# hbdat/cvpr22_cross_modal_pseudo_labeling

Measured on AMD Instinct MI355X. Metric: images/sec student-teacher train step (COCO 800x1333), higher is better.
Workload: dtype f32 (bf16x3 split MFMA, fp32 accum); 1 GPU; student_teacher_mask_rcnn_uncertainty.yaml R-50-C4, 2 img/GPU 3x800x1333, fwd+bwd+allreduce+SGD; global_batch=2, parallelism=dp1, losses_finite=True, pipelined=True

## Files before the change

cvpr22_cross_modal_pseudo_labeling_amd/csrc/ovis_common.h:

```cpp
#pragma once
#include <hip/hip_runtime.h>
#include <stdint.h>

#include "ovis_hip.h"

#define OVIS_HIP_TRY(expr)                         \
  do {                                             \
    hipError_t _e = (expr);                        \
    if (_e != hipSuccess) return (int)_e;          \
  } while (0)

#define OVIS_LAUNCH_CHECK()                        \
  do {                                             \
    hipError_t _e = hipGetLastError();             \
    if (_e != hipSuccess) return (int)_e;          \
  } while (0)

static inline int ovis_ceil_div(long a, long b) { return (int)((a + b - 1) / b); }

#define OVIS_NUM_CU 256
#define OVIS_WAVE 64
```

cvpr22_cross_modal_pseudo_labeling_amd/csrc/split_gemm.hip:

```cpp
#include <stdlib.h>

#include "ovis_common.h"
constexpr int kGroupWidth = 4;

namespace {
typedef short bf16x8 __attribute__((ext_vector_type(8)));
typedef float f32x4 __attribute__((ext_vector_type(4)));
typedef __bf16 b2 __attribute__((ext_vector_type(2)));
typedef float f2 __attribute__((ext_vector_type(2)));

__device__ char g_zero_line[128];

enum { PLAIN = 0, SHIFTED = 1, HALO = 2, DEFORM = 3 };
constexpr int kHalo = 8;

struct SplitGemmArgs {
  const char* A; long a_rs;
  const char* A2; long a2_rs;
  const char* B; long b_rs;
  float* C; long ldc;
  char* Cp; long cp_rs;
  const float* bias; const float* res; long ldr;
  const char* resp; long resp_rs;
  const char* gate; long gate_rs;
  float* pool; int pool_rows; float pool_scale;
  float* slab;
  long M; int N; int ch; int ch2; int T; int H; int W; int KH; int KW; int flip; int relu; int gw;
  int kslices; int steps_per_slice;
  const float* dimg; const float* doff; const float* dmask;
  int Ho; int Wo; int sh; int sw; int ph; int pw; int dlh; int dlw; int dg;
};

__device__ __forceinline__ void glds16(const char* gsrc, char* lds_wave_base) {
  __builtin_amdgcn_global_load_lds((const __attribute__((address_space(1))) void*)gsrc,
                                   (__attribute__((address_space(3))) void*)lds_wave_base, 16, 0, 0);
}

__device__ __forceinline__ unsigned pack_bf16(float a, float b) {
  f2 v = {a, b};
  return __builtin_bit_cast(unsigned, __builtin_convertvector(v, b2));
}

struct EpilogueOperands {
  uint2 a, b;
};

struct EpilogueSource {
  const char* base;
  long row_bytes;
  int second;
};

__device__ __forceinline__ EpilogueSource epilogue_source(const SplitGemmArgs& p) {
// ... 427 lines not shown
            if constexpr (POOL) {
              const int rr = f * 16 + r;
              const f32x4 z = {0.f, 0.f, 0.f, 0.f};
              ps0 += rr < pool_b1 ? fin : z;
              ps1 += (rr >= pool_b1 && rr < pool_b2) ? fin : z;
              ps2 += rr >= pool_b2 ? fin : z;
            }
          }
        }
      }
    }
  }
  if constexpr (POOL) {
    f32x4* ps[3] = {&ps0, &ps1, &ps2};
#pragma unroll
    for (int sgm = 0; sgm < 3; ++sgm) {
      f32x4 v = *ps[sgm];
#pragma unroll
      for (int e = 0; e < 4; ++e) {
        v[e] += __shfl_xor(v[e], 16, 64);
        v[e] += __shfl_xor(v[e], 32, 64);
      }
      const long first = (m0 + wm * 64) + (sgm == 0 ? 0 : (sgm == 1 ? pool_b1 : pool_b2));
      if (er == 0 && col_ok && first < p.M && (sgm == 0 || (sgm == 1 ? pool_b1 : pool_b2) < 64)) {
        float* d = p.pool + (pool_map0 + sgm) * p.N + n;
#pragma unroll
        for (int e = 0; e < 4; ++e) atomicAdd(d + e, v[e] * p.pool_scale);
      }
    }
  }
}

__global__ __launch_bounds__(256) void split_gemm_finish_kernel(SplitGemmArgs p) {
  const int n4 = p.N >> 2;
  const long total = p.M * n4;
  const long slab = p.M * p.N;
  for (long i = (long)blockIdx.x * 256 + threadIdx.x; i < total; i += (long)gridDim.x * 256) {
    const long m = i / n4;
    const int n = (int)(i - m * n4) * 4;
    const float* s = p.slab + m * p.N + n;
    f32x4 v = *(const f32x4*)s;
    for (int k = 1; k < p.kslices; ++k) v += *(const f32x4*)(s + k * slab);
    epilogue_store4(p, m, n, v);
  }
}

typedef short bf16x4 __attribute__((ext_vector_type(4)));

struct SplitGemmTnArgs {
  const char* G; long g_rs;
  const char* X; long x_rs;
  float* C;
  long M; int N; int ch; int T; int H; int W; int KH; int KW; int slices; int steps_per_slice;
  int g_major;
};

#define OVIS_TR_READ(dst, addr, off) \
  asm volatile("ds_read_b64_tr_b16 %0, %1 offset:%2" : "=v"(dst) : "v"(addr), "n"(off) : "memory")
#define OVIS_LGKM_WAIT8(N, a, b, c, d, e, f, g, h)                                                                \
  asm volatile("s_waitcnt lgkmcnt(%8)"                                                                             \
               : "+v"(a), "+v"(b), "+v"(c), "+v"(d), "+v"(e), "+v"(f), "+v"(g), "+v"(h)                            \
               : "n"(N)                                                                                            \
               : "memory")

template <bool CONV, bool SMALL = false>
__global__ __launch_bounds__(256, 2) void split_gemm_tn_kernel(SplitGemmTnArgs p, int tiles_i, int tiles_j,
                                                              int nblocks) {
  constexpr int TILE_BYTES = 32 * 512, STAGE = 2 * TILE_BYTES;
  extern __shared__ __attribute__((aligned(16))) char smem[];
  const int lane = threadIdx.x & 63, wave = threadIdx.x >> 6;
  int id;
  {
    constexpr int kChunk = 2 * OVIS_NUM_CU;
    const int b = blockIdx.x, base = b / kChunk * kChunk;
    const int nb = min(nblocks - base, kChunk), bl = b - base;
    const int q = nb >> 3, r = nb & 7, xcd = bl & 7, loc = bl >> 3;
    id = base + (xcd < r ? xcd * (q + 1) : r * (q + 1) + (xcd - r) * q) + loc;
  }
  const int per_slice = tiles_i * tiles_j;
  const int slice = id / per_slice;
  const int rem = id - slice * per_slice;
  const int tile_j = p.g_major ? rem % tiles_j : rem / tiles_i;
  const int tile_i = p.g_major ? rem / tiles_j : rem - tile_j * tiles_i;
  const int i0 = tile_i * 128, j0 = tile_j * 128;
  const int tap = CONV ? j0 / p.ch : 0, c0 = CONV ? j0 - tap * p.ch : j0;
  int off_rows = 0, tdy = 0, tdx = 0;
  if (CONV) {
    tdy = tap / p.KW - p.KH / 2;
    tdx = tap % p.KW - p.KW / 2;
    off_rows = tdy * p.W + tdx;
  }
  const long step0 = (long)slice * p.steps_per_slice;
  const long steps_total = (p.M + 31) >> 5;
  long step1 = step0 + p.steps_per_slice;
  if (step1 > steps_total) step1 = steps_total;
  const int nk = step1 > step0 ? (int)(step1 - step0) : 0;

  const int prow = lane >> 5, pseg = (lane & 31) >> 1, phalf = lane & 1;
  int rows[4];
  long g_off[4], x_off[4];
  int x_y[4], x_x[4];
  int m_row[4];
  const int HW = CONV ? p.H * p.W : 1;
  unsigned long long tap_mask = 0;
  if (CONV && SMALL) {
    const int qy = lane / p.W, qx = lane - qy * p.W;
    tap_mask = __ballot(lane < HW && (unsigned)(qy + tdy) < (unsigned)p.H && (unsigned)(qx + tdx) < (unsigned)p.W);
  }
#pragma unroll
  for (int i = 0; i < 4; ++i) {
    const int piece = wave * 4 + i;
    const int row = piece * 2 + prow;
    rows[i] = row;
    const int fr = (((row >> 3) & 1) << 2) | (row & 3);
    const int seg = pseg ^ fr;
    const int m = (int)(step0 << 5) + row;
    m_row[i] = m;
    g_off[i] = (long)m * p.g_rs + (long)i0 * 4 + seg * 32 + phalf * 16;
    x_off[i] = ((long)m + off_rows) * p.x_rs + (long)c0 * 4 + seg * 32 + phalf * 16;
    x_x[i] = CONV ? (SMALL ? m % HW : m % p.W) : 0;
    x_y[i] = (CONV && !SMALL) ? (m / p.W) % p.H : 0;
  }
  const int step_q = (CONV && SMALL) ? 32 % HW : 0;
  const int step_dx = CONV ? 32 % p.W : 0, step_dy = CONV ? 32 / p.W : 0;
  const bool y_single = step_dy + 1 <= p.H;
  const char* zero_src = g_zero_line + (lane & 7) * 16;
  const int Mi = (int)p.M;

  auto issue = [&](int stage) {
    char* base = smem + stage * STAGE;
    bool x_ok[4];
#pragma unroll
    for (int i = 0; i < 4; ++i) {
      x_ok[i] = m_row[i] < Mi;
      if (CONV && SMALL) {
        x_ok[i] = x_ok[i] && ((tap_mask >> x_x[i]) & 1ull) != 0ull;
        int q = x_x[i] + step_q;
        if (q >= HW) q -= HW;
        x_x[i] = q;
      } else if (CONV) {
        x_ok[i] = x_ok[i] && (unsigned)(x_y[i] + tdy) < (unsigned)p.H && (unsigned)(x_x[i] + tdx) < (unsigned)p.W;
        int x = x_x[i] + step_dx, y = x_y[i] + step_dy;
        if (x >= p.W) { x -= p.W; ++y; }
        if (y_single) { if (y >= p.H) y -= p.H; } else { y %= p.H; }
        x_x[i] = x;
        x_y[i] = y;
      }
    }
#pragma unroll
    for (int i = 0; i < 4; ++i) {
      const char* src = p.G + g_off[i];
      if (m_row[i] >= Mi) src = zero_src;
      glds16(src, base + (wave * 4 + i) * 1024);
      g_off[i] += 32 * p.g_rs;
    }
#pragma unroll
    for (int i = 0; i < 4; ++i) {
      const char* src = p.X + x_off[i];
      if (!x_ok[i]) src = zero_src;
      glds16(src, base + TILE_BYTES + (wave * 4 + i) * 1024);
      x_off[i] += 32 * p.x_rs;
      m_row[i] += 32;
    }
  };

  const int wi = wave >> 1, wj = wave & 1;
  const int gq = lane >> 4, pp = lane & 15;
  const int rrow = 8 * gq + (pp >> 2);
  const int rfr = ((gq & 1) << 2) | (pp >> 2);
  int g_rd[4], x_rd[4];
#pragma unroll
  for (int f = 0; f < 4; ++f) {
    const int seg_g = (2 * wi + (f >> 1)) * 4 + (f & 1);
    g_rd[f] = rrow * 512 + ((seg_g ^ rfr) << 5) + (pp & 3) * 8;
    const int seg_x = (2 * wj + (f >> 1)) * 4 + (f & 1);
    x_rd[f] = TILE_BYTES + rrow * 512 + ((seg_x ^ rfr) << 5) + (pp & 3) * 8;
  }

  f32x4 acc[4][4];
#pragma unroll
  for (int f = 0; f < 4; ++f)
#pragma unroll
    for (int g = 0; g < 4; ++g) acc[f][g] = f32x4{0.f, 0.f, 0.f, 0.f};

  if (nk > 0) issue(0);
  for (int kb = 0; kb < nk; ++kb) {
    __syncthreads();
    if (kb + 1 < nk) issue((kb + 1) & 1);
    const int so = (kb & 1) * STAGE;
    bf16x4 xa[4][2], xb[4][2], ga[4][2], gb[4][2];
#pragma unroll
    for (int f = 0; f < 4; ++f) {
      const int ax = so + x_rd[f], ag = so + g_rd[f];
      OVIS_TR_READ(xa[f][0], ax, 0);
      OVIS_TR_READ(xb[f][0], ax, 2048);
      OVIS_TR_READ(ga[f][0], ag, 0);
      OVIS_TR_READ(gb[f][0], ag, 2048);
    }
#pragma unroll
    for (int f = 0; f < 4; ++f) {
      const int ax = so + (x_rd[f] ^ 64), ag = so + (g_rd[f] ^ 64);
      OVIS_TR_READ(xa[f][1], ax, 0);
      OVIS_TR_READ(xb[f][1], ax, 2048);
      OVIS_TR_READ(ga[f][1], ag, 0);
      OVIS_TR_READ(gb[f][1], ag, 2048);
    }
    OVIS_LGKM_WAIT8(15, xa[0][0], xb[0][0], ga[0][0], gb[0][0], xa[1][0], xb[1][0], ga[1][0], gb[1][0]);
    OVIS_LGKM_WAIT8(15, xa[2][0], xb[2][0], ga[2][0], gb[2][0], xa[3][0], xb[3][0], ga[3][0], gb[3][0]);
    bf16x8 gh[4], gl[4], xh[4], xl[4];
#pragma unroll
    for (int f = 0; f < 4; ++f) {
      xh[f] = __builtin_shufflevector(xa[f][0], xb[f][0], 0, 1, 2, 3, 4, 5, 6, 7);
      gh[f] = __builtin_shufflevector(ga[f][0], gb[f][0], 0, 1, 2, 3, 4, 5, 6, 7);
    }
#pragma unroll
    for (int f = 0; f < 4; ++f)
#pragma unroll
      for (int g = 0; g < 4; ++g)
        acc[f][g] = __builtin_amdgcn_mfma_f32_16x16x32_bf16(xh[g], gh[f], acc[f][g], 0, 0, 0);
    OVIS_LGKM_WAIT8(0, xa[0][1], xb[0][1], ga[0][1], gb[0][1], xa[1][1], xb[1][1], ga[1][1], gb[1][1]);
    OVIS_LGKM_WAIT8(0, xa[2][1], xb[2][1], ga[2][1], gb[2][1], xa[3][1], xb[3][1], ga[3][1], gb[3][1]);
#pragma unroll
    for (int f = 0; f < 4; ++f) {
      xl[f] = __builtin_shufflevector(xa[f][1], xb[f][1], 0, 1, 2, 3, 4, 5, 6, 7);
      gl[f] = __builtin_shufflevector(ga[f][1], gb[f][1], 0, 1, 2, 3, 4, 5, 6, 7);
    }
#pragma unroll
    for (int f = 0; f < 4; ++f)
#pragma unroll
      for (int g = 0; g < 4; ++g)
        acc[f][g] = __builtin_amdgcn_mfma_f32_16x16x32_bf16(xh[g], gl[f], acc[f][g], 0, 0, 0);
#pragma unroll
    for (int f = 0; f < 4; ++f)
#pragma unroll
      for (int g = 0; g < 4; ++g)
        acc[f][g] = __builtin_amdgcn_mfma_f32_16x16x32_bf16(xl[g], gh[f], acc[f][g], 0, 0, 0);
  }

  const long ld = (long)p.T * p.ch;
  float* out = p.C + (long)slice * p.N * ld;
#pragma unroll
// ... 350 lines not shown

extern "C" int ovis_split_gemm_tn_slices(long m, int n, int channels, int taps) {
  if (m <= 0 || n <= 0 || channels <= 0 || taps <= 0) return 1;
  const long tiles = (long)(n / 128) * ((long)taps * channels / 128);
  const long steps = (m + 31) / 32;
  if (tiles <= 0) return 1;
  const long slots = 2L * OVIS_NUM_CU;
  if (steps >= 128 && steps <= 1100 && tiles <= 64) {
    long s = slots / tiles;
    if (s > steps / 16) s = steps / 16;
    if (s > 256) s = 256;
    return (int)(s < 1 ? 1 : s);
  }
  long s_max = (4 * slots + tiles - 1) / tiles;
  if (s_max > steps / 8) s_max = steps / 8;
  if (s_max > 256) s_max = 256;
  if (s_max < 1) s_max = 1;
  long best = 1;
  double best_score = -1.0;
  for (long s = 1; s <= s_max; ++s) {
    const long blocks = s * tiles, rounds = (blocks + slots - 1) / slots;
    double score = (double)blocks / (double)(rounds * slots);
    if (rounds == 1) score *= 0.97 * (double)blocks / (double)slots;
    if (rounds > 2) score -= 0.01 * (double)(rounds - 2);
    if (score > best_score + 1e-9) { best_score = score; best = s; }
  }
  return (int)best;
}

extern "C" int ovis_split_gemm_pair_tn(const void* g_pair, long g_row_bytes, const void* x_pair, long x_row_bytes,
                                       float* c_slabs, int slices, long m, int n, int channels, int taps_h,
                                       int taps_w, int height, int width, void* stream) {
  if (m < 0 || n <= 0 || channels <= 0 || taps_h <= 0 || taps_w <= 0 || !(taps_h & 1) || !(taps_w & 1) || slices <= 0)
    return OVIS_EINVAL;
  if (!g_pair || !x_pair || !c_slabs || m > 0x7fffff00L) return OVIS_EINVAL;
  const int T = taps_h * taps_w;
  if (T > 1 && (height <= 0 || width <= 0)) return OVIS_EINVAL;
  if (n % 128 != 0 || channels % 128 != 0 ||
      g_row_bytes % 16 != 0 || x_row_bytes % 16 != 0 || ((uintptr_t)g_pair & 15) || ((uintptr_t)x_pair & 15) ||
      ((uintptr_t)c_slabs & 15))
    return OVIS_ERANGE;
  SplitGemmTnArgs p;
  p.G = (const char*)g_pair; p.g_rs = g_row_bytes; p.X = (const char*)x_pair; p.x_rs = x_row_bytes;
  p.C = c_slabs; p.M = m; p.N = n; p.ch = channels; p.T = T; p.H = height; p.W = width; p.KH = taps_h; p.KW = taps_w;
  p.slices = slices;
  const long steps = (m + 31) / 32;
  p.steps_per_slice = (int)((steps + slices - 1) / slices);
  const int tiles_i = n / 128, tiles_j = (int)((long)T * channels / 128);
  p.g_major = tiles_i >= channels / 128 ? 1 : 0;
  const long nblocks = (long)tiles_i * tiles_j * slices;
  if (nblocks > 0x7fffffffL) return OVIS_ERANGE;
  hipStream_t s = (hipStream_t)stream;
  const int lds = 2 * 2 * 32 * 512;
  if (T > 1 && (long)height * width <= 64) {
    static bool attr_set_s = false;
    if (!attr_set_s) {
      OVIS_HIP_TRY(hipFuncSetAttribute((const void*)split_gemm_tn_kernel<true, true>, hipFuncAttributeMaxDynamicSharedMemorySize, lds));
      attr_set_s = true;
    }
    hipLaunchKernelGGL((split_gemm_tn_kernel<true, true>), dim3((unsigned)nblocks), dim3(256), lds, s, p, tiles_i, tiles_j, (int)nblocks);
  } else if (T > 1) {
    static bool attr_set_c = false;
    if (!attr_set_c) {
      OVIS_HIP_TRY(hipFuncSetAttribute((const void*)split_gemm_tn_kernel<true>, hipFuncAttributeMaxDynamicSharedMemorySize, lds));
      attr_set_c = true;
    }
    hipLaunchKernelGGL(split_gemm_tn_kernel<true>, dim3((unsigned)nblocks), dim3(256), lds, s, p, tiles_i, tiles_j, (int)nblocks);
  } else {
    static bool attr_set = false;
    if (!attr_set) {
      OVIS_HIP_TRY(hipFuncSetAttribute((const void*)split_gemm_tn_kernel<false>, hipFuncAttributeMaxDynamicSharedMemorySize, lds));
      attr_set = true;
    }
    hipLaunchKernelGGL(split_gemm_tn_kernel<false>, dim3((unsigned)nblocks), dim3(256), lds, s, p, tiles_i, tiles_j, (int)nblocks);
  }
  OVIS_LAUNCH_CHECK();
  return OVIS_OK;
}

namespace {
struct SplitGemmPlan {
  int mode, narrow, stages, kslices, steps_per_slice, tiles_m, tiles_n;
};

SplitGemmPlan split_gemm_plan(long m, int n, int channels, int channels2, int taps_h, int taps_w, int width, int config) {
  SplitGemmPlan q;
  const int T = taps_h * taps_w;
  q.narrow = n <= 64;
  const int bn = q.narrow ? 64 : 128;
  q.tiles_m = (int)((m + 127) / 128);
  q.tiles_n = (n + bn - 1) / bn;
  const long nb = (long)q.tiles_m * q.tiles_n;
  q.mode = PLAIN;
  if (T > 1) q.mode = (!q.narrow && !(config & 4) && (taps_h / 2) * width + taps_w / 2 <= kHalo && T <= 16) ? HALO : SHIFTED;
  const int cpb = channels / 32;
  const int units = q.mode == HALO ? cpb : T * cpb + channels2 / 32;
  q.kslices = 1;
  q.steps_per_slice = units;
  bool sliced_two_stage = false;
  if (!(config & 8) && !q.narrow && nb <= OVIS_NUM_CU / 2) {
    const int min_units = q.mode == HALO ? 1 : 8;
    long s = units / min_units;
    const long want = (2L * OVIS_NUM_CU + nb - 1) / nb;
    if (s > want) s = want;
    if (s > 64) s = 64;
    if (s >= 2) {
      q.steps_per_slice = (int)((units + s - 1) / s);
// ... 275 lines not shown
```

cvpr22_cross_modal_pseudo_labeling_amd/csrc/roi_align.hip:

```cpp
#include <stdlib.h>

#include "ovis_common.h"
#include "roi_geom.h"

namespace {
using namespace ovis_roi;

constexpr int kThreads = 256;
constexpr int kCPB = 32;
constexpr int kMaxBatch = 16;
constexpr int kFwdLdsFloats = 4352;


template <int NCS>
__device__ __forceinline__ void fwd_pool(const float* src, int cs, int rs, int oy, int ox,
                                         const RoiGeom& g, int H, int W, int PH, int PW,
                                         float* __restrict__ out_c0) {
  const int PHPW = PH * PW;
  for (int bin = threadIdx.x; bin < PHPW; bin += kThreads) {
    const int ph = bin / PW;
    const int pw = bin - ph * PW;
    float acc[NCS];
#pragma unroll
    for (int c = 0; c < NCS; ++c) acc[c] = 0.f;
// ... 253 lines not shown
    t_xrow = (t_bin - ph * PW) * g.gw;
  }
  while (c < c_end) {
    const int left = c_end - c;
    const float* plane = img + (long)c * HW;
    float* o = out_r + (long)c * PHPW;
    const int n = min(left, cs_max);
    if (tables && n >= 16) {
      fwd_batch_lds4_tab<16>(win, plane, HW, W, g, wh, ww, PHPW, ytab, xtab, t_bin, t_yrow, t_xrow, o);
      c += 16;
    } else if (tables && n >= 8) {
      fwd_batch_lds4_tab<8>(win, plane, HW, W, g, wh, ww, PHPW, ytab, xtab, t_bin, t_yrow, t_xrow, o);
      c += 8;
    } else if (tables && n >= 4) {
      fwd_batch_lds4_tab<4>(win, plane, HW, W, g, wh, ww, PHPW, ytab, xtab, t_bin, t_yrow, t_xrow, o);
      c += 4;
    } else if (n >= 16) {
      fwd_batch_lds4<16>(win, plane, HW, W, H, g, wh, ww, PH, PW, o);
      c += 16;
    } else if (n >= 8) {
      fwd_batch_lds4<8>(win, plane, HW, W, H, g, wh, ww, PH, PW, o);
      c += 8;
    } else if (n >= 4) {
      fwd_batch_lds4<4>(win, plane, HW, W, H, g, wh, ww, PH, PW, o);
      c += 4;
    } else if (n >= 2) {
      fwd_batch_lds<2>(win, plane, HW, W, H, g, wh, ww, PH, PW, o);
      c += 2;
    } else if (n == 1) {
      fwd_batch_lds<1>(win, plane, HW, W, H, g, wh, ww, PH, PW, o);
      c += 1;
    } else {
      fwd_pool<1>(plane, HW, W, 0, 0, g, H, W, PH, PW, o);
      c += 1;
    }
  }
}

typedef __bf16 pool_b2 __attribute__((ext_vector_type(2)));
typedef float pool_f2 __attribute__((ext_vector_type(2)));
__device__ __forceinline__ unsigned pool_pack_bf16(float a, float b) {
  pool_f2 v = {a, b};
  return __builtin_bit_cast(unsigned, __builtin_convertvector(v, pool_b2));
}
__device__ __forceinline__ void pool_store4_pair(char* pair_r, long obin, int c, int C, f4 o) {
  const unsigned h01 = pool_pack_bf16(o.x, o.y), h23 = pool_pack_bf16(o.z, o.w);
  const unsigned l01 = pool_pack_bf16(o.x - __uint_as_float(h01 << 16), o.y - __uint_as_float(h01 & 0xffff0000u));
  const unsigned l23 = pool_pack_bf16(o.z - __uint_as_float(h23 << 16), o.w - __uint_as_float(h23 & 0xffff0000u));
  char* d = pair_r + obin * 4L * C + (long)(c >> 5) * 128 + (c & 31) * 2;
  *(uint2*)d = make_uint2(h01, h23);
  *(uint2*)(d + 64) = make_uint2(l01, l23);
}

template <int NCS, bool FAST>
__device__ __forceinline__ void fwd_pool4_strided(const f4* win4, int rs, const RoiGeom& g, int H, int W, int bs,
                                                  int OH, int OW, float* __restrict__ out_rc, int C,
                                                  char* pair_r = nullptr, int c_abs = 0) {
  constexpr int NG = NCS / 4;
  constexpr int SG = kFwdLdsFloats / NCS;
  const int items = OH * OW * NG;
  for (int item = threadIdx.x; item < items; item += kThreads) {
    const int k = item % NG, obin = item / NG;
    const int oh = obin / OW;
    const int ph = oh * bs, pw = (obin - oh * OW) * bs;
    const f4* base = win4 + k * SG;
    f4 acc = (f4)(0.f);
    for (int iy = 0; iy < g.gh; ++iy) {
      const float y = sample_coord_t<FAST>(g.start_h, ph, g.bin_h, iy, g.gh, g.inv_gh);
      int yl, yh;
      float ly, hy;
      if (!axis_sample(y, H, yl, yh, ly, hy)) continue;
      const int ryl = (yl - g.wy0) * rs, ryh = (yh - g.wy0) * rs;
      for (int ix = 0; ix < g.gw; ++ix) {
        const float x = sample_coord_t<FAST>(g.start_w, pw, g.bin_w, ix, g.gw, g.inv_gw);
        int xl, xh;
        float lx, hx;
        if (!axis_sample(x, W, xl, xh, lx, hx)) continue;
        const float w1 = hy * hx, w2 = hy * lx, w3 = ly * hx, w4 = ly * lx;
        acc += w1 * base[ryl + (xl - g.wx0)] + w2 * base[ryl + (xh - g.wx0)] + w3 * base[ryh + (xl - g.wx0)] +
               w4 * base[ryh + (xh - g.wx0)];
      }
    }
    const f4 o = FAST ? acc * g.inv_count : acc / g.count;
    if (pair_r) pool_store4_pair(pair_r, obin, c_abs + 4 * k, C, o);
    else *(f4*)(out_rc + (long)obin * C + 4 * k) = o;
  }
}

template <bool FAST>
__device__ __forceinline__ void pool_nhwc_strided(const f4* __restrict__ img4, const RoiGeom& g, int H, int W, int C4,
                                                  int bs, int OH, int OW, float* __restrict__ out_r, char* pair_r,
                                                  int k0 = 0, int KT = -1) {
  if (KT < 0) KT = C4;
  const int items = OH * OW * KT;
  const int C = C4 * 4;
  if (g.gh == 2 && g.gw == 2) {
    for (int item = threadIdx.x; item < items; item += kThreads) {
      const int k = k0 + item % KT, obin = item / KT;
      const int oh = obin / OW;
      const int ph = oh * bs, pw = (obin - oh * OW) * bs;
      const f4* base = img4 + k;
      int yl[2], yh[2], xl[2], xh[2];
      float ly[2], hy[2], lx[2], hx[2];
      bool oky[2], okx[2];
#pragma unroll
      for (int i = 0; i < 2; ++i) {
        oky[i] = axis_sample(sample_coord_t<FAST>(g.start_h, ph, g.bin_h, i, 2, g.inv_gh), H, yl[i], yh[i], ly[i], hy[i]);
        okx[i] = axis_sample(sample_coord_t<FAST>(g.start_w, pw, g.bin_w, i, 2, g.inv_gw), W, xl[i], xh[i], lx[i], hx[i]);
      }
      const bool same_rows = oky[0] && oky[1] && yl[0] == yl[1] && yh[0] == yh[1];
      const bool same_cols = okx[0] && okx[1] && xl[0] == xl[1] && xh[0] == xh[1];
      f4 t[2][2][4];
      auto load4 = [&](int iy, int ix) {
        const long ryl = (long)yl[iy] * W * C4, ryh = (long)yh[iy] * W * C4;
        const long cl = (long)xl[ix] * C4, ch = (long)xh[ix] * C4;
        t[iy][ix][0] = base[ryl + cl];
        t[iy][ix][1] = base[ryl + ch];
        t[iy][ix][2] = base[ryh + cl];
        t[iy][ix][3] = base[ryh + ch];
      };
      auto copy4 = [&](int iy, int ix, int sy, int sx) {
#pragma unroll
        for (int q = 0; q < 4; ++q) t[iy][ix][q] = t[sy][sx][q];
      };
      if (oky[0] && okx[0]) load4(0, 0);
      if (oky[0] && okx[1]) { if (same_cols) copy4(0, 1, 0, 0); else load4(0, 1); }
      if (oky[1] && okx[0]) { if (same_rows) copy4(1, 0, 0, 0); else load4(1, 0); }
      if (oky[1] && okx[1]) {
        if (same_rows) copy4(1, 1, 0, 1);
        else if (same_cols) copy4(1, 1, 1, 0);
        else load4(1, 1);
      }
      f4 acc = (f4)(0.f);
#pragma unroll
      for (int iy = 0; iy < 2; ++iy) {
        if (!oky[iy]) continue;
#pragma unroll
        for (int ix = 0; ix < 2; ++ix) {
          if (!okx[ix]) continue;
          const float w1 = hy[iy] * hx[ix], w2 = hy[iy] * lx[ix], w3 = ly[iy] * hx[ix], w4 = ly[iy] * lx[ix];
          acc += w1 * t[iy][ix][0] + w2 * t[iy][ix][1] + w3 * t[iy][ix][2] + w4 * t[iy][ix][3];
// ... 5 lines not shown
    }
    return;
  }
  for (int item = threadIdx.x; item < items; item += kThreads) {
    const int k = k0 + item % KT, obin = item / KT;
    const int oh = obin / OW;
    const int ph = oh * bs, pw = (obin - oh * OW) * bs;
    const f4* base = img4 + k;
    f4 acc = (f4)(0.f);
    for (int iy = 0; iy < g.gh; ++iy) {
      const float y = sample_coord_t<FAST>(g.start_h, ph, g.bin_h, iy, g.gh, g.inv_gh);
      int yl, yh;
      float ly, hy;
      if (!axis_sample(y, H, yl, yh, ly, hy)) continue;
      const long ryl = (long)yl * W * C4, ryh = (long)yh * W * C4;
      for (int ix = 0; ix < g.gw; ++ix) {
        const float x = sample_coord_t<FAST>(g.start_w, pw, g.bin_w, ix, g.gw, g.inv_gw);
        int xl, xh;
        float lx, hx;
        if (!axis_sample(x, W, xl, xh, lx, hx)) continue;
        const float w1 = hy * hx, w2 = hy * lx, w3 = ly * hx, w4 = ly * lx;
        const long cl = (long)xl * C4, ch = (long)xh * C4;
        acc += w1 * base[ryl + cl] + w2 * base[ryl + ch] + w3 * base[ryh + cl] + w4 * base[ryh + ch];
      }
    }
    const f4 o = FAST ? acc * g.inv_count : acc / g.count;
    if (pair_r) pool_store4_pair(pair_r, obin, 4 * k, C, o);
    else *(f4*)(out_r + (long)obin * C + 4 * k) = o;
  }
}

__global__ __launch_bounds__(kThreads) void roi_align_fwd_nhwc_in_strided_kernel(
    const float* __restrict__ in, const float* __restrict__ rois, float* __restrict__ out, int R, int batch, int C,
    int H, int W, int PH, int PW, int bs, int OH, int OW, float scale, int sampling_ratio, int pair_out) {
  const int r = blockIdx.x;
  const RoiGeom g = make_geom(rois + (long)r * 5, scale, H, W, PH, PW, sampling_ratio, batch);
  float* out_r = out + (long)r * OH * OW * C;
  char* pair_r = pair_out ? (char*)out_r : nullptr;
  const int C4 = C >> 2;
  if (g.empty) {
    for (int item = threadIdx.x; item < OH * OW * C4; item += kThreads) {
      const int k = item % C4, obin = item / C4;
      if (pair_r) pool_store4_pair(pair_r, obin, 4 * k, C, (f4)(0.f));
      else *(f4*)(out_r + (long)obin * C + 4 * k) = (f4)(0.f);
    }
    return;
  }
  const f4* img4 = (const f4*)(in + (long)g.b * H * W * C);
  if (g.pow2) pool_nhwc_strided<true>(img4, g, H, W, C4, bs, OH, OW, out_r, pair_r);
  else pool_nhwc_strided<false>(img4, g, H, W, C4, bs, OH, OW, out_r, pair_r);
}

constexpr int kSmallWindow = 272;

template <int NCS>
__device__ __forceinline__ void stage_window4_nhwc(float* win, const float* __restrict__ img_c0, int C, int W,
                                                   const RoiGeom& g, int wh, int ww) {
  constexpr int NG = NCS / 4;
  constexpr int SG = kFwdLdsFloats / NCS;
  f4* win4 = (f4*)win;
  const int n = wh * ww * NG;
  const float inv_ww = 1.f / (float)ww;
  for (int i = threadIdx.x; i < n; i += kThreads) {
    const int k = i % NG, idx = i / NG;
    const int y = (int)(((float)idx + 0.5f) * inv_ww);
    const int x = idx - y * ww;
    win4[k * SG + idx] = *(const f4*)(img_c0 + ((long)(g.wy0 + y) * W + (g.wx0 + x)) * C + 4 * k);
  }
}

template <int NCS>
__device__ __forceinline__ void strided_batch4_nhwc(float* win, const float* __restrict__ img_c0, int C, int H, int W,
                                                    const RoiGeom& g, int wh, int ww, int bs, int OH, int OW,
                                                    float* __restrict__ out_rc, char* pair_r, int c_abs) {
  stage_window4_nhwc<NCS>(win, img_c0, C, W, g, wh, ww);
  __syncthreads();
  if (g.pow2)
    fwd_pool4_strided<NCS, true>((const f4*)win, ww, g, H, W, bs, OH, OW, out_rc, C, pair_r, c_abs);
  else
    fwd_pool4_strided<NCS, false>((const f4*)win, ww, g, H, W, bs, OH, OW, out_rc, C, pair_r, c_abs);
  __syncthreads();
}

__global__ __launch_bounds__(kThreads) void roi_align_fwd_nhwc_in_strided_lds_kernel(
    const float* __restrict__ in, const float* __restrict__ rois, float* __restrict__ out, int R, int batch, int C,
    int H, int W, int PH, int PW, int bs, int OH, int OW, float scale, int sampling_ratio, int pair_out) {
  __shared__ __attribute__((aligned(16))) float win[kFwdLdsFloats];
  const int r = blockIdx.x % R;
  const int ct = blockIdx.x / R;
  const int c_begin = ct * kCPB;
  const RoiGeom g = make_geom(rois + (long)r * 5, scale, H, W, PH, PW, sampling_ratio, batch);
  float* out_r = out + (long)r * OH * OW * C;
  char* pair_r = pair_out ? (char*)out_r : nullptr;
  if (g.empty) {
    for (int item = threadIdx.x; item < OH * OW * (kCPB / 4); item += kThreads) {
      const int k = item % (kCPB / 4), obin = item / (kCPB / 4);
      if (pair_r) pool_store4_pair(pair_r, obin, c_begin + 4 * k, C, (f4)(0.f));
      else *(f4*)(out_r + (long)obin * C + c_begin + 4 * k) = (f4)(0.f);
    }
    return;
  }
  const int wh = g.wy1 - g.wy0 + 1, ww = g.wx1 - g.wx0 + 1;
  const int warea = wh * ww;
  const float* img = in + (long)g.b * H * W * C;
  if (warea > kSmallWindow) {
    if (g.pow2) pool_nhwc_strided<true>((const f4*)img, g, H, W, C >> 2, bs, OH, OW, out_r, pair_r, c_begin >> 2, kCPB / 4);
    else pool_nhwc_strided<false>((const f4*)img, g, H, W, C >> 2, bs, OH, OW, out_r, pair_r, c_begin >> 2, kCPB / 4);
    return;
  }
  if (warea * 32 <= kFwdLdsFloats) {
    strided_batch4_nhwc<32>(win, img + c_begin, C, H, W, g, wh, ww, bs, OH, OW, out_r + c_begin, pair_r, c_begin);
  } else {
    strided_batch4_nhwc<16>(win, img + c_begin, C, H, W, g, wh, ww, bs, OH, OW, out_r + c_begin, pair_r, c_begin);
    strided_batch4_nhwc<16>(win, img + c_begin + 16, C, H, W, g, wh, ww, bs, OH, OW, out_r + c_begin + 16, pair_r,
                            c_begin + 16);
  }
}


template <int NCS>
__device__ __forceinline__ void bwd_batch(const float* Ay, const float* Ax, const int* phlo,
                                          const int* phhi, const int* pwlo, const int* pwhi,
                                          float* G, const float* __restrict__ gout_c0,
                                          float* __restrict__ gin_c0, int HW, int W,
                                          const RoiGeom& g, int wh, int ww, int PH, int PW) {
  const int PHPW = PH * PW;
  const int n = NCS * PHPW;
  for (int i = threadIdx.x; i < n; i += kThreads) G[i] = gout_c0[i];
  __syncthreads();
  const int warea = wh * ww;
  const float inv_ww = 1.f / (float)ww;
  for (int idx = threadIdx.x; idx < warea; idx += kThreads) {
    const int y = (int)(((float)idx + 0.5f) * inv_ww);
    const int x = idx - y * ww;
    const int p0 = phlo[y], p1 = phhi[y], q0 = pwlo[x], q1 = pwhi[x];
    if (p1 < p0 || q1 < q0) continue;
    float s[NCS];
#pragma unroll
    for (int c = 0; c < NCS; ++c) s[c] = 0.f;
    for (int ph = p0; ph <= p1; ++ph) {
      const float ay = Ay[ph * wh + y];
      for (int pw = q0; pw <= q1; ++pw) {
        const float w = ay * Ax[pw * ww + x];
        const float* gp = G + ph * PW + pw;
#pragma unroll
        for (int c = 0; c < NCS; ++c) s[c] += w * gp[c * PHPW];
      }
    }
    float* dst = gin_c0 + (long)(g.wy0 + y) * W + (g.wx0 + x);
#pragma unroll
    for (int c = 0; c < NCS; ++c) atomicAdd(dst + (long)c * HW, s[c] / g.count);
  }
  __syncthreads();
}

__global__ __launch_bounds__(kThreads) void roi_align_bwd_kernel(
    const float* __restrict__ gout, const float* __restrict__ rois, float* __restrict__ gin,
    int R, int batch, int C, int H, int W, int PH, int PW, float scale, int sampling_ratio) {
  extern __shared__ __attribute__((aligned(16))) float smem[];
  float* Ay = smem;
  float* Ax = Ay + PH * H;
  int* phlo = (int*)(Ax + PW * W);
  int* phhi = phlo + H;
  int* pwlo = phhi + H;
  int* pwhi = pwlo + W;
  float* G = (float*)(pwhi + W);

  const int r = blockIdx.x % R;
  const int ct = blockIdx.x / R;
// ... 209 lines not shown
  return rc == -100 ? OVIS_ERANGE : rc;
}

extern "C" int ovis_roi_align_backward_strided_nhwc_ws_f32(const float* grad_output_nhwc, const float* rois,
                                                           float* grad_input, int num_rois, int batch, int channels,
                                                           int height, int width, int pooled_h, int pooled_w,
                                                           int bin_stride, float spatial_scale, int sampling_ratio,
                                                           void* workspace, size_t workspace_bytes, void* stream) {
  if (num_rois < 0 || batch < 0 || channels < 0 || height <= 0 || width <= 0 || pooled_h <= 0 || pooled_w <= 0 ||
      bin_stride <= 0)
    return OVIS_EINVAL;
  if ((size_t)batch * channels == 0) return OVIS_OK;
  if (!grad_input) return OVIS_EINVAL;
  if (num_rois == 0)
    return (int)hipMemsetAsync(grad_input, 0, (size_t)batch * channels * height * width * sizeof(float), (hipStream_t)stream);
  const int th = (pooled_h + bin_stride - 1) / bin_stride, tw = (pooled_w + bin_stride - 1) / bin_stride;
  if (th > 8 || tw > 8 || !ovis_roi_align_backward_plane_supported(height, width, th, tw)) return OVIS_ERANGE;
  if (!grad_output_nhwc || !rois) return OVIS_EINVAL;
  const int rc = ovis_roi_align_backward_plane_launch(grad_output_nhwc, rois, grad_input, num_rois, batch, channels, height,
                                                      width, pooled_h, pooled_w, bin_stride, spatial_scale,
                                                      sampling_ratio, workspace, workspace_bytes, (hipStream_t)stream, 1);
  return rc == -100 ? OVIS_ERANGE : rc;
}

extern "C" int ovis_roi_align_forward_ws_f32(const float* input, const float* rois, float* output, int num_rois,
                                             int batch, int channels, int height, int width, int pooled_h,
                                             int pooled_w, float spatial_scale, int sampling_ratio, void* workspace,
                                             size_t workspace_bytes, void* stream) {
  if (num_rois < 0 || batch < 0 || channels < 0 || height <= 0 || width <= 0 || pooled_h <= 0 || pooled_w <= 0)
    return OVIS_EINVAL;
  if (num_rois == 0 || channels == 0) return OVIS_OK;
  if (!input || !rois || !output) return OVIS_EINVAL;
  if (ovis_roi_align_forward_mfma_supported(height, width, pooled_h, pooled_w))
    return ovis_roi_align_forward_mfma_launch(input, rois, output, num_rois, batch, channels, height, width, pooled_h,
                                              pooled_w, spatial_scale, sampling_ratio, workspace, workspace_bytes,
                                              (hipStream_t)stream);
  return ovis_roi_align_forward_f32(input, rois, output, num_rois, batch, channels, height, width, pooled_h, pooled_w,
                                    spatial_scale, sampling_ratio, stream);
}

extern "C" int ovis_roi_align_forward_strided_from_nhwc_f32(const float* input_nhwc, const float* rois, void* output,
                                                            int num_rois, int batch, int channels, int height,
                                                            int width, int pooled_h, int pooled_w, int bin_stride,
                                                            float spatial_scale, int sampling_ratio, int pair_out,
                                                            void* stream) {
  if (num_rois < 0 || batch < 0 || channels < 0 || height <= 0 || width <= 0 || pooled_h <= 0 || pooled_w <= 0 ||
      bin_stride <= 0)
    return OVIS_EINVAL;
  if (num_rois == 0 || channels == 0) return OVIS_OK;
  if (!input_nhwc || !rois || !output) return OVIS_EINVAL;
  if (channels % 4 != 0 || (pair_out && channels % 32 != 0) || ((uintptr_t)input_nhwc & 15) || ((uintptr_t)output & 15))
    return OVIS_ERANGE;
  const int oh = (pooled_h + bin_stride - 1) / bin_stride, ow = (pooled_w + bin_stride - 1) / bin_stride;
  const long tiles = (long)(channels / kCPB) * num_rois;
  const int kCoResidencyPadBytes = pair_out ? 40 * 1024 : 0;
  if (channels % kCPB == 0 && tiles <= 0x7fffffffL)
    hipLaunchKernelGGL(roi_align_fwd_nhwc_in_strided_lds_kernel, dim3((unsigned)tiles), dim3(kThreads), kCoResidencyPadBytes,
                       (hipStream_t)stream, input_nhwc, rois, (float*)output, num_rois, batch, channels, height, width,
                       pooled_h, pooled_w, bin_stride, oh, ow, spatial_scale, sampling_ratio, pair_out);
  else
    hipLaunchKernelGGL(roi_align_fwd_nhwc_in_strided_kernel, dim3((unsigned)num_rois), dim3(kThreads), 0, (hipStream_t)stream,
                       input_nhwc, rois, (float*)output, num_rois, batch, channels, height, width, pooled_h, pooled_w,
                       bin_stride, oh, ow, spatial_scale, sampling_ratio, pair_out);
  OVIS_LAUNCH_CHECK();
  return OVIS_OK;
}
```

Baseline: 60.21 images/sec.

## Walk only valid tap pixels in small-map conv weight-gradient GEMM

For convolution weight-gradient GEMMs on small feature maps (H*W<=64, e.g. ROI heads), the K loop now iterates only over pixels whose shifted tap stays in bounds, rather than over every pixel with out-of-bounds rows zero-filled. A magic-multiply tap walker maps the compacted index back to a pixel row, and row addresses are computed with a single mad_u64_u32. This removes zero-padding loads and MFMA work for border taps, at the cost of extra per-row index arithmetic and tighter launch preconditions (m divisible by H*W, 32-bit strides).

```diff
diff --git a/cvpr22_cross_modal_pseudo_labeling_amd/csrc/ovis_common.h b/cvpr22_cross_modal_pseudo_labeling_amd/csrc/ovis_common.h
--- a/cvpr22_cross_modal_pseudo_labeling_amd/csrc/ovis_common.h
+++ b/cvpr22_cross_modal_pseudo_labeling_amd/csrc/ovis_common.h
@@ -20,3 +20,46 @@
 
 #define OVIS_NUM_CU 256
 #define OVIS_WAVE 64
+
+struct OvisTapWalk {
+  int nv;
+  int wv;
+  int magic;
+  int wgap;
+  int pix0;
+};
+
+__host__ __device__ static inline OvisTapWalk ovis_tap_walk(int H, int W, int tdy, int tdx) {
+  OvisTapWalk t;
+  const int y0 = tdy < 0 ? -tdy : 0, x0 = tdx < 0 ? -tdx : 0;
+  const int hv = H - (tdy < 0 ? -tdy : tdy), wv = W - (tdx < 0 ? -tdx : tdx);
+  const bool any = hv > 0 && wv > 0;
+  t.nv = any ? hv * wv : 0;
+  t.wv = any ? wv : 1;
+  t.magic = (65536 + t.wv - 1) / t.wv;
+  t.wgap = W - t.wv;
+  t.pix0 = y0 * W + x0;
+  return t;
+}
+
+__host__ __device__ static inline unsigned ovis_mul24(unsigned a, unsigned b) { return (a & 0xffffffu) * (b & 0xffffffu); }
+
+__host__ __device__ static inline int ovis_tap_walk_pixel(const OvisTapWalk& t, int q) {
+  const unsigned yy = ovis_mul24((unsigned)q, (unsigned)t.magic) >> 16;
+  return t.pix0 + q + (int)ovis_mul24(yy, (unsigned)t.wgap);
+}
+
+__host__ __device__ static inline void ovis_tap_walk_seek(const OvisTapWalk& t, unsigned c, int& r, int& q) {
+  r = (int)(c / (unsigned)t.nv);
+  q = (int)(c - (unsigned)r * (unsigned)t.nv);
+}
+
+__host__ __device__ static inline void ovis_tap_walk_advance(const OvisTapWalk& t, int step_mb, int step_q, int HW, int& mb,
+                                                             int& q) {
+  q += step_q;
+  mb += step_mb;
+  if (q >= t.nv) {
+    q -= t.nv;
+    mb += HW;
+  }
+}
diff --git a/cvpr22_cross_modal_pseudo_labeling_amd/csrc/split_gemm.hip b/cvpr22_cross_modal_pseudo_labeling_amd/csrc/split_gemm.hip
--- a/cvpr22_cross_modal_pseudo_labeling_amd/csrc/split_gemm.hip
+++ b/cvpr22_cross_modal_pseudo_labeling_amd/csrc/split_gemm.hip
@@ -1,4 +1,6 @@
 #include <stdlib.h>
+
+#include <type_traits>
 
 #include "ovis_common.h"
 constexpr int kGroupWidth = 4;
@@ -532,6 +534,7 @@
   const char* X; long x_rs;
   float* C;
   long M; int N; int ch; int T; int H; int W; int KH; int KW; int slices; int steps_per_slice;
+  int R;
   int g_major;
 };
 
@@ -542,6 +545,12 @@
                : "+v"(a), "+v"(b), "+v"(c), "+v"(d), "+v"(e), "+v"(f), "+v"(g), "+v"(h)                            \
                : "n"(N)                                                                                            \
                : "memory")
+
+__device__ __forceinline__ const char* tn_row_address(const char* base, unsigned row, unsigned stride) {
+  unsigned long long out;
+  asm("v_mad_u64_u32 %0, vcc, %1, %2, %3" : "=&v"(out) : "v"(row), "s"(stride), "v"((unsigned long long)base) : "vcc");
+  return (const char*)out;
+}
 
 template <bool CONV, bool SMALL = false>
 __global__ __launch_bounds__(256, 2) void split_gemm_tn_kernel(SplitGemmTnArgs p, int tiles_i, int tiles_j,
@@ -570,9 +579,20 @@
     tdx = tap % p.KW - p.KW / 2;
     off_rows = tdy * p.W + tdx;
   }
-  const long step0 = (long)slice * p.steps_per_slice;
-  const long steps_total = (p.M + 31) >> 5;
-  long step1 = step0 + p.steps_per_slice;
+  const int HW = CONV ? p.H * p.W : 1;
+  const OvisTapWalk tw = ovis_tap_walk((CONV && SMALL) ? p.H : 1, (CONV && SMALL) ? p.W : 1, tdy, tdx);
+  long step0, steps_total;
+  int per_slice_steps;
+  if (CONV && SMALL) {
+    const int steps_t = (int)(((long)p.R * tw.nv + 31) >> 5);
+    per_slice_steps = (steps_t + p.slices - 1) / p.slices;
+    steps_total = steps_t;
+  } else {
+    per_slice_steps = p.steps_per_slice;
+    steps_total = (p.M + 31) >> 5;
+  }
+  step0 = (long)slice * per_slice_steps;
+  long step1 = step0 + per_slice_steps;
   if (step1 > steps_total) step1 = steps_total;
   const int nk = step1 > step0 ? (int)(step1 - step0) : 0;
 
@@ -581,12 +601,8 @@
   long g_off[4], x_off[4];
   int x_y[4], x_x[4];
   int m_row[4];
-  const int HW = CONV ? p.H * p.W : 1;
-  unsigned long long tap_mask = 0;
-  if (CONV && SMALL) {
-    const int qy = lane / p.W, qx = lane - qy * p.W;
-    tap_mask = __ballot(lane < HW && (unsigned)(qy + tdy) < (unsigned)p.H && (unsigned)(qx + tdx) < (unsigned)p.W);
-  }
+  const char *g_base[4], *x_base[4];
+  int w_mb[4], w_q[4];
 #pragma unroll
   for (int i = 0; i < 4; ++i) {
     const int piece = wave * 4 + i;
@@ -598,27 +614,51 @@
     m_row[i] = m;
     g_off[i] = (long)m * p.g_rs + (long)i0 * 4 + seg * 32 + phalf * 16;
     x_off[i] = ((long)m + off_rows) * p.x_rs + (long)c0 * 4 + seg * 32 + phalf * 16;
-    x_x[i] = CONV ? (SMALL ? m % HW : m % p.W) : 0;
-    x_y[i] = (CONV && !SMALL) ? (m / p.W) % p.H : 0;
-  }
-  const int step_q = (CONV && SMALL) ? 32 % HW : 0;
+    x_x[i] = CONV ? m % p.W : 0;
+    x_y[i] = CONV ? (m / p.W) % p.H : 0;
+    if (CONV && SMALL) {
+      g_base[i] = p.G + ((long)i0 * 4 + seg * 32 + phalf * 16);
+      x_base[i] = p.X + ((long)off_rows * p.x_rs + (long)c0 * 4 + seg * 32 + phalf * 16);
+      int r = 0;
+      w_q[i] = 0;
+      if (nk > 0) ovis_tap_walk_seek(tw, (unsigned)m, r, w_q[i]);
+      w_mb[i] = r * HW;
+    }
+  }
+  const int step_mb = (CONV && SMALL && tw.nv > 0) ? 32 / tw.nv * HW : 0, step_q = (CONV && SMALL && tw.nv > 0) ? 32 % tw.nv : 0;
+  const unsigned g_rs32 = (unsigned)p.g_rs, x_rs32 = (unsigned)p.x_rs;
   const int step_dx = CONV ? 32 % p.W : 0, step_dy = CONV ? 32 / p.W : 0;
   const bool y_single = step_dy + 1 <= p.H;
   const char* zero_src = g_zero_line + (lane & 7) * 16;
   const int Mi = (int)p.M;
 
-  auto issue = [&](int stage) {
+  auto issue_as = [&](int stage, auto tail) {
     char* base = smem + stage * STAGE;
+    if (CONV && SMALL) {
+      const char *gs[4], *xs[4];
+#pragma unroll
+      for (int i = 0; i < 4; ++i) {
+        unsigned mrow = (unsigned)(w_mb[i] + ovis_tap_walk_pixel(tw, w_q[i]));
+        const char *gb = g_base[i], *xb = x_base[i];
+        if (tail() && w_mb[i] >= Mi) {
+          mrow = 0;
+          gb = xb = zero_src;
+        }
+        gs[i] = tn_row_address(gb, mrow, g_rs32);
+        xs[i] = tn_row_address(xb, mrow, x_rs32);
+        ovis_tap_walk_advance(tw, step_mb, step_q, HW, w_mb[i], w_q[i]);
+      }
+#pragma unroll
+      for (int i = 0; i < 4; ++i) glds16(gs[i], base + (wave * 4 + i) * 1024);
+#pragma unroll
+      for (int i = 0; i < 4; ++i) glds16(xs[i], base + TILE_BYTES + (wave * 4 + i) * 1024);
+      return;
+    }
     bool x_ok[4];
 #pragma unroll
     for (int i = 0; i < 4; ++i) {
       x_ok[i] = m_row[i] < Mi;
-      if (CONV && SMALL) {
-        x_ok[i] = x_ok[i] && ((tap_mask >> x_x[i]) & 1ull) != 0ull;
-        int q = x_x[i] + step_q;
-        if (q >= HW) q -= HW;
-        x_x[i] = q;
-      } else if (CONV) {
+      if (CONV) {
         x_ok[i] = x_ok[i] && (unsigned)(x_y[i] + tdy) < (unsigned)p.H && (unsigned)(x_x[i] + tdx) < (unsigned)p.W;
         int x = x_x[i] + step_dx, y = x_y[i] + step_dy;
         if (x >= p.W) { x -= p.W; ++y; }
@@ -644,6 +684,11 @@
     }
   };
 
+  auto issue = [&](int stage, bool tail) {
+    if ((CONV && SMALL) && tail) issue_as(stage, std::true_type());
+    else issue_as(stage, std::false_type());
+  };
+
   const int wi = wave >> 1, wj = wave & 1;
   const int gq = lane >> 4, pp = lane & 15;
   const int rrow = 8 * gq + (pp >> 2);
@@ -663,10 +708,10 @@
 #pragma unroll
     for (int g = 0; g < 4; ++g) acc[f][g] = f32x4{0.f, 0.f, 0.f, 0.f};
 
-  if (nk > 0) issue(0);
+  if (nk > 0) issue(0, step0 + 1 == steps_total);
   for (int kb = 0; kb < nk; ++kb) {
     __syncthreads();
-    if (kb + 1 < nk) issue((kb + 1) & 1);
+    if (kb + 1 < nk) issue((kb + 1) & 1, step0 + kb + 2 == steps_total);
     const int so = (kb & 1) * STAGE;
     bf16x4 xa[4][2], xb[4][2], ga[4][2], gb[4][2];
 #pragma unroll
@@ -1123,7 +1168,10 @@
   if (nblocks > 0x7fffffffL) return OVIS_ERANGE;
   hipStream_t s = (hipStream_t)stream;
   const int lds = 2 * 2 * 32 * 512;
-  if (T > 1 && (long)height * width <= 64) {
+  const bool small_maps = T > 1 && (long)height * width <= 64 && m % ((long)height * width) == 0 && m <= 0x7fff0000L && g_row_bytes > 0 &&
+                          g_row_bytes <= 0x7fffffffL && x_row_bytes > 0 && x_row_bytes <= 0x7fffffffL;
+  p.R = small_maps ? (int)(m / ((long)height * width)) : 0;
+  if (small_maps) {
     static bool attr_set_s = false;
     if (!attr_set_s) {
       OVIS_HIP_TRY(hipFuncSetAttribute((const void*)split_gemm_tn_kernel<true, true>, hipFuncAttributeMaxDynamicSharedMemorySize, lds));
```

New measurement: 60.99 images/sec, median of 6. 1.3% higher.

## Process channel slabs per block with double-buffered LDS and precomputed sample tables

Applied to the files above, without the earlier changes.

The strided NHWC ROIAlign forward now has each block handle a slab of several 32-channel tiles for one ROI, not a single tile. The next channel group's window is loaded into registers while the current one is pooled from a double-buffered LDS window. Per-axis bilinear sample indices and weights are computed once into small LDS tables and reused across channel groups. The goal is less repeated geometry math and block launch overhead, and hiding global load latency. In exchange it doubles static LDS and raises register pressure, which can lower occupancy.

```diff
diff --git a/cvpr22_cross_modal_pseudo_labeling_amd/csrc/roi_align.hip b/cvpr22_cross_modal_pseudo_labeling_amd/csrc/roi_align.hip
--- a/cvpr22_cross_modal_pseudo_labeling_amd/csrc/roi_align.hip
+++ b/cvpr22_cross_modal_pseudo_labeling_amd/csrc/roi_align.hip
@@ -329,41 +329,6 @@
   *(uint2*)(d + 64) = make_uint2(l01, l23);
 }
 
-template <int NCS, bool FAST>
-__device__ __forceinline__ void fwd_pool4_strided(const f4* win4, int rs, const RoiGeom& g, int H, int W, int bs,
-                                                  int OH, int OW, float* __restrict__ out_rc, int C,
-                                                  char* pair_r = nullptr, int c_abs = 0) {
-  constexpr int NG = NCS / 4;
-  constexpr int SG = kFwdLdsFloats / NCS;
-  const int items = OH * OW * NG;
-  for (int item = threadIdx.x; item < items; item += kThreads) {
-    const int k = item % NG, obin = item / NG;
-    const int oh = obin / OW;
-    const int ph = oh * bs, pw = (obin - oh * OW) * bs;
-    const f4* base = win4 + k * SG;
-    f4 acc = (f4)(0.f);
-    for (int iy = 0; iy < g.gh; ++iy) {
-      const float y = sample_coord_t<FAST>(g.start_h, ph, g.bin_h, iy, g.gh, g.inv_gh);
-      int yl, yh;
-      float ly, hy;
-      if (!axis_sample(y, H, yl, yh, ly, hy)) continue;
-      const int ryl = (yl - g.wy0) * rs, ryh = (yh - g.wy0) * rs;
-      for (int ix = 0; ix < g.gw; ++ix) {
-        const float x = sample_coord_t<FAST>(g.start_w, pw, g.bin_w, ix, g.gw, g.inv_gw);
-        int xl, xh;
-        float lx, hx;
-        if (!axis_sample(x, W, xl, xh, lx, hx)) continue;
-        const float w1 = hy * hx, w2 = hy * lx, w3 = ly * hx, w4 = ly * lx;
-        acc += w1 * base[ryl + (xl - g.wx0)] + w2 * base[ryl + (xh - g.wx0)] + w3 * base[ryh + (xl - g.wx0)] +
-               w4 * base[ryh + (xh - g.wx0)];
-      }
-    }
-    const f4 o = FAST ? acc * g.inv_count : acc / g.count;
-    if (pair_r) pool_store4_pair(pair_r, obin, c_abs + 4 * k, C, o);
-    else *(f4*)(out_rc + (long)obin * C + 4 * k) = o;
-  }
-}
-
 template <bool FAST>
 __device__ __forceinline__ void pool_nhwc_strided(const f4* __restrict__ img4, const RoiGeom& g, int H, int W, int C4,
                                                   int bs, int OH, int OW, float* __restrict__ out_r, char* pair_r,
@@ -475,49 +440,154 @@
 }
 
 constexpr int kSmallWindow = 272;
-
-template <int NCS>
-__device__ __forceinline__ void stage_window4_nhwc(float* win, const float* __restrict__ img_c0, int C, int W,
-                                                   const RoiGeom& g, int wh, int ww) {
+constexpr int kTabCap = 64;
+constexpr int kStageSlots = (kFwdLdsFloats / 4 + kThreads - 1) / kThreads;
+constexpr int kSlabMinGrid = 1024;
+
+struct __attribute__((aligned(16))) AxisEntry { int lo, hi; float l, h; };
+
+template <int NCS, bool FAST, int GF>
+__device__ __forceinline__ void fwd_pool4_strided_tab(const f4* win4, const AxisEntry* ytab, const AxisEntry* xtab,
+                                                      const RoiGeom& g, int OH, int OW, float inv_ow,
+                                                      float* __restrict__ out_rc, int C, char* pair_r, int c_abs) {
+  constexpr int NG = NCS / 4;
+  constexpr int SG = kFwdLdsFloats / NCS;
+  const int gh = GF ? GF : g.gh, gw = GF ? GF : g.gw;
+  const int items = OH * OW * NG;
+  for (int item = threadIdx.x; item < items; item += kThreads) {
+    const int k = item % NG, obin = item / NG;
+    const int oh = (int)(((float)obin + 0.5f) * inv_ow);
+    const int ow = obin - oh * OW;
+    const f4* base = win4 + k * SG;
+    const AxisEntry* ty = ytab + oh * gh;
+    const AxisEntry* tx = xtab + ow * gw;
+    f4 acc = (f4)(0.f);
+    for (int iy = 0; iy < gh; ++iy) {
+      const AxisEntry ey = ty[iy];
+      if (ey.lo < 0) continue;
+      const int ryl = ey.lo, ryh = ey.hi;
+      const float ly = ey.l, hy = ey.h;
+      for (int ix = 0; ix < gw; ++ix) {
+        const AxisEntry ex = tx[ix];
+        if (ex.lo < 0) continue;
+        const int xl = ex.lo, xh = ex.hi;
+        const float lx = ex.l, hx = ex.h;
+        const float w1 = hy * hx, w2 = hy * lx, w3 = ly * hx, w4 = ly * lx;
+        acc += w1 * base[ryl + xl] + w2 * base[ryl + xh] + w3 * base[ryh + xl] +
+               w4 * base[ryh + xh];
+      }
+    }
+    const f4 o = FAST ? acc * g.inv_count : acc / g.count;
+    if (pair_r) pool_store4_pair(pair_r, obin, c_abs + 4 * k, C, o);
+    else *(f4*)(out_rc + (long)obin * C + 4 * k) = o;
+  }
+}
+
+template <int NCS, bool FAST, int GF>
+__device__ __forceinline__ void strided_slab_nhwc(float* win, const AxisEntry* ytab, const AxisEntry* xtab,
+                                                  const float* __restrict__ img_c0, int nch, int C, int W,
+                                                  const RoiGeom& g, int wh, int ww, int OH, int OW,
+                                                  float* __restrict__ out_rc, char* pair_r, int c_abs) {
   constexpr int NG = NCS / 4;
   constexpr int SG = kFwdLdsFloats / NCS;
   f4* win4 = (f4*)win;
+  const int T = nch / NCS;
   const int n = wh * ww * NG;
-  const float inv_ww = 1.f / (float)ww;
-  for (int i = threadIdx.x; i < n; i += kThreads) {
+  const float inv_ww = 1.f / (float)ww, inv_ow = 1.f / (float)OW;
+  long goff[kStageSlots];
+  bool act[kStageSlots];
+  int loff[kStageSlots];
+  f4 pre[kStageSlots];
+#pragma unroll
+  for (int j = 0; j < kStageSlots; ++j) {
+    const int i = threadIdx.x + j * kThreads;
     const int k = i % NG, idx = i / NG;
     const int y = (int)(((float)idx + 0.5f) * inv_ww);
     const int x = idx - y * ww;
-    win4[k * SG + idx] = *(const f4*)(img_c0 + ((long)(g.wy0 + y) * W + (g.wx0 + x)) * C + 4 * k);
-  }
-}
-
-template <int NCS>
-__device__ __forceinline__ void strided_batch4_nhwc(float* win, const float* __restrict__ img_c0, int C, int H, int W,
-                                                    const RoiGeom& g, int wh, int ww, int bs, int OH, int OW,
-                                                    float* __restrict__ out_rc, char* pair_r, int c_abs) {
-  stage_window4_nhwc<NCS>(win, img_c0, C, W, g, wh, ww);
-  __syncthreads();
-  if (g.pow2)
-    fwd_pool4_strided<NCS, true>((const f4*)win, ww, g, H, W, bs, OH, OW, out_rc, C, pair_r, c_abs);
+    act[j] = i < n;
+    goff[j] = act[j] ? ((long)(g.wy0 + y) * W + (g.wx0 + x)) * C + 4 * k : 0L;
+    loff[j] = k * SG + idx;
+  }
+  auto load = [&](int t) {
+#pragma unroll
+    for (int j = 0; j < kStageSlots; ++j)
+      pre[j] = *(const f4*)(img_c0 + t * NCS + goff[j]);
+  };
+  auto store = [&](f4* buf) {
+#pragma unroll
+    for (int j = 0; j < kStageSlots; ++j)
+      if (act[j]) buf[loff[j]] = pre[j];
+  };
+  load(0);
+  store(win4);
+  if (T > 1) load(1);
+  __syncthreads();
+  for (int t = 0; t < T; ++t) {
+    fwd_pool4_strided_tab<NCS, FAST, GF>(win4 + (t & 1) * (kFwdLdsFloats / 4), ytab, xtab, g, OH, OW, inv_ow,
+                                         out_rc + t * NCS, C, pair_r, c_abs + t * NCS);
+    if (t + 1 < T) {
+      store(win4 + ((t + 1) & 1) * (kFwdLdsFloats / 4));
+      if (t + 2 < T) load(t + 2);
+    }
+    __syncthreads();
+  }
+}
+
+template <bool FAST, int GF>
+__device__ __forceinline__ void strided_tables_slab_nhwc(float* win, AxisEntry* ytab, AxisEntry* xtab,
+                                                         const float* __restrict__ img_c0, int nch, int C, int H, int W,
+                                                         const RoiGeom& g, int wh, int ww, int bs, int OH, int OW,
+                                                         float* __restrict__ out_rc, char* pair_r, int c_abs) {
+  const int e = threadIdx.x & 63;
+  if (threadIdx.x < 64) {
+    if (e < OH * g.gh) {
+      const int oh = e / g.gh, iy = e - oh * g.gh;
+      const int ph = oh * bs;
+      const float y = sample_coord_t<FAST>(g.start_h, ph, g.bin_h, iy, g.gh, g.inv_gh);
+      int yl, yh;
+      float ly, hy;
+      AxisEntry t = {-1, -1, 0.f, 0.f};
+      if (axis_sample(y, H, yl, yh, ly, hy)) t = {(yl - g.wy0) * ww, (yh - g.wy0) * ww, ly, hy};
+      ytab[e] = t;
+    }
+  } else if (threadIdx.x < 128) {
+    if (e < OW * g.gw) {
+      const int ow = e / g.gw, ix = e - ow * g.gw;
+      const int pw = ow * bs;
+      const float x = sample_coord_t<FAST>(g.start_w, pw, g.bin_w, ix, g.gw, g.inv_gw);
+      int xl, xh;
+      float lx, hx;
+      AxisEntry t = {-1, -1, 0.f, 0.f};
+      if (axis_sample(x, W, xl, xh, lx, hx)) t = {xl - g.wx0, xh - g.wx0, lx, hx};
+      xtab[e] = t;
+    }
+  }
+  const int warea = wh * ww;
+  if (warea * 64 <= kFwdLdsFloats && nch % 64 == 0)
+    strided_slab_nhwc<64, FAST, GF>(win, ytab, xtab, img_c0, nch, C, W, g, wh, ww, OH, OW, out_rc, pair_r, c_abs);
+  else if (warea * 32 <= kFwdLdsFloats)
+    strided_slab_nhwc<32, FAST, GF>(win, ytab, xtab, img_c0, nch, C, W, g, wh, ww, OH, OW, out_rc, pair_r, c_abs);
   else
-    fwd_pool4_strided<NCS, false>((const f4*)win, ww, g, H, W, bs, OH, OW, out_rc, C, pair_r, c_abs);
-  __syncthreads();
+    strided_slab_nhwc<16, FAST, GF>(win, ytab, xtab, img_c0, nch, C, W, g, wh, ww, OH, OW, out_rc, pair_r, c_abs);
 }
 
 __global__ __launch_bounds__(kThreads) void roi_align_fwd_nhwc_in_strided_lds_kernel(
     const float* __restrict__ in, const float* __restrict__ rois, float* __restrict__ out, int R, int batch, int C,
-    int H, int W, int PH, int PW, int bs, int OH, int OW, float scale, int sampling_ratio, int pair_out) {
-  __shared__ __attribute__((aligned(16))) float win[kFwdLdsFloats];
+    int H, int W, int PH, int PW, int bs, int OH, int OW, float scale, int sampling_ratio, int pair_out,
+    int slab_tiles) {
+  __shared__ __attribute__((aligned(16))) float win[2 * kFwdLdsFloats];
+  __shared__ AxisEntry ytab[kTabCap], xtab[kTabCap];
   const int r = blockIdx.x % R;
-  const int ct = blockIdx.x / R;
-  const int c_begin = ct * kCPB;
+  const int t_begin = (blockIdx.x / R) * slab_tiles;
+  const int c_begin = t_begin * kCPB;
+  const int nch = min(slab_tiles, C / kCPB - t_begin) * kCPB;
   const RoiGeom g = make_geom(rois + (long)r * 5, scale, H, W, PH, PW, sampling_ratio, batch);
   float* out_r = out + (long)r * OH * OW * C;
   char* pair_r = pair_out ? (char*)out_r : nullptr;
   if (g.empty) {
-    for (int item = threadIdx.x; item < OH * OW * (kCPB / 4); item += kThreads) {
-      const int k = item % (kCPB / 4), obin = item / (kCPB / 4);
+    const int KG = nch / 4;
+    for (int item = threadIdx.x; item < OH * OW * KG; item += kThreads) {
+      const int k = item % KG, obin = item / KG;
       if (pair_r) pool_store4_pair(pair_r, obin, c_begin + 4 * k, C, (f4)(0.f));
       else *(f4*)(out_r + (long)obin * C + c_begin + 4 * k) = (f4)(0.f);
     }
@@ -526,18 +596,21 @@
   const int wh = g.wy1 - g.wy0 + 1, ww = g.wx1 - g.wx0 + 1;
   const int warea = wh * ww;
   const float* img = in + (long)g.b * H * W * C;
-  if (warea > kSmallWindow) {
-    if (g.pow2) pool_nhwc_strided<true>((const f4*)img, g, H, W, C >> 2, bs, OH, OW, out_r, pair_r, c_begin >> 2, kCPB / 4);
-    else pool_nhwc_strided<false>((const f4*)img, g, H, W, C >> 2, bs, OH, OW, out_r, pair_r, c_begin >> 2, kCPB / 4);
+  const bool tables_fit = g.gh <= kTabCap && g.gw <= kTabCap && OH * g.gh <= kTabCap && OW * g.gw <= kTabCap;
+  if (warea > kSmallWindow || !tables_fit) {
+    if (g.pow2) pool_nhwc_strided<true>((const f4*)img, g, H, W, C >> 2, bs, OH, OW, out_r, pair_r, c_begin >> 2, nch / 4);
+    else pool_nhwc_strided<false>((const f4*)img, g, H, W, C >> 2, bs, OH, OW, out_r, pair_r, c_begin >> 2, nch / 4);
     return;
   }
-  if (warea * 32 <= kFwdLdsFloats) {
-    strided_batch4_nhwc<32>(win, img + c_begin, C, H, W, g, wh, ww, bs, OH, OW, out_r + c_begin, pair_r, c_begin);
-  } else {
-    strided_batch4_nhwc<16>(win, img + c_begin, C, H, W, g, wh, ww, bs, OH, OW, out_r + c_begin, pair_r, c_begin);
-    strided_batch4_nhwc<16>(win, img + c_begin + 16, C, H, W, g, wh, ww, bs, OH, OW, out_r + c_begin + 16, pair_r,
-                            c_begin + 16);
-  }
+  if (g.gh == 2 && g.gw == 2)
+    strided_tables_slab_nhwc<true, 2>(win, ytab, xtab, img + c_begin, nch, C, H, W, g, wh, ww, bs, OH, OW,
+                                      out_r + c_begin, pair_r, c_begin);
+  else if (g.pow2)
+    strided_tables_slab_nhwc<true, 0>(win, ytab, xtab, img + c_begin, nch, C, H, W, g, wh, ww, bs, OH, OW,
+                                      out_r + c_begin, pair_r, c_begin);
+  else
+    strided_tables_slab_nhwc<false, 0>(win, ytab, xtab, img + c_begin, nch, C, H, W, g, wh, ww, bs, OH, OW,
+                                       out_r + c_begin, pair_r, c_begin);
 }
 
 
@@ -853,12 +926,15 @@
   if (channels % 4 != 0 || (pair_out && channels % 32 != 0) || ((uintptr_t)input_nhwc & 15) || ((uintptr_t)output & 15))
     return OVIS_ERANGE;
   const int oh = (pooled_h + bin_stride - 1) / bin_stride, ow = (pooled_w + bin_stride - 1) / bin_stride;
-  const long tiles = (long)(channels / kCPB) * num_rois;
+  const int ctiles = channels / kCPB;
+  int slab_tiles = 8;
+  while (slab_tiles > 2 && (long)num_rois * ((ctiles + slab_tiles - 1) / slab_tiles) < kSlabMinGrid) slab_tiles >>= 1;
+  const long tiles = (long)((ctiles + slab_tiles - 1) / slab_tiles) * num_rois;
   const int kCoResidencyPadBytes = pair_out ? 40 * 1024 : 0;
   if (channels % kCPB == 0 && tiles <= 0x7fffffffL)
     hipLaunchKernelGGL(roi_align_fwd_nhwc_in_strided_lds_kernel, dim3((unsigned)tiles), dim3(kThreads), kCoResidencyPadBytes,
                        (hipStream_t)stream, input_nhwc, rois, (float*)output, num_rois, batch, channels, height, width,
-                       pooled_h, pooled_w, bin_stride, oh, ow, spatial_scale, sampling_ratio, pair_out);
+                       pooled_h, pooled_w, bin_stride, oh, ow, spatial_scale, sampling_ratio, pair_out, slab_tiles);
   else
     hipLaunchKernelGGL(roi_align_fwd_nhwc_in_strided_kernel, dim3((unsigned)num_rois), dim3(kThreads), 0, (hipStream_t)stream,
                        input_nhwc, rois, (float*)output, num_rois, batch, channels, height, width, pooled_h, pooled_w,
```

Result: no change. 59.90 images/sec before, 60.36 images/sec after (median of 6 runs) (+0.8%).
